# hila-chefer/Transformer-Explainability

Hardware: NVIDIA H100
Metric: explanations_per_sec (higher is better)
Workload: dtype f32

## Files before the change

transformer_explainability_b200/csrc/te_tc_wgmma.cu:

```cuda
#include <cuda.h>
#include <cuda_bf16.h>
#include <cuda_fp16.h>
#include <cuda_runtime.h>
#include <string.h>
#include <algorithm>
#include <string>
#include <type_traits>
#include <utility>

#include "te_gemm_tc.h"
#include "te_wgmma.cuh"

namespace {

constexpr int BM = 128, NTHREADS = 256;

__device__ __forceinline__ uint32_t smem_u32(const void* p) { return (uint32_t)__cvta_generic_to_shared(p); }
__device__ __forceinline__ void fence_proxy_async() { asm volatile("fence.proxy.async.shared::cta;" ::: "memory"); }
__device__ __forceinline__ void wg_fence() { asm volatile("wgmma.fence.sync.aligned;" ::: "memory"); }
__device__ __forceinline__ void wg_commit() { asm volatile("wgmma.commit_group.sync.aligned;" ::: "memory"); }
__device__ __forceinline__ void wg_wait0() { asm volatile("wgmma.wait_group.sync.aligned 0;" ::: "memory"); }
__device__ __forceinline__ void wg_wait1() { asm volatile("wgmma.wait_group.sync.aligned 1;" ::: "memory"); }

__device__ __forceinline__ void mbar_init(uint32_t bar, uint32_t count) {
    asm volatile("mbarrier.init.shared::cta.b64 [%0], %1;" ::"r"(bar), "r"(count) : "memory");
}
__device__ __forceinline__ void mbar_expect_tx(uint32_t bar, uint32_t bytes) {
    asm volatile("mbarrier.arrive.expect_tx.shared::cta.b64 _, [%0], %1;" ::"r"(bar), "r"(bytes) : "memory");
}
__device__ __forceinline__ void mbar_arrive(uint32_t bar) { asm volatile("mbarrier.arrive.shared::cta.b64 _, [%0];" ::"r"(bar) : "memory"); }
__device__ __forceinline__ void mbar_wait(uint32_t bar, uint32_t parity) {
    uint32_t done;
    do {
        asm volatile("{\n.reg .pred p;\nmbarrier.try_wait.parity.shared::cta.b64 p, [%1], %2;\nselp.u32 %0, 1, 0, p;\n}\n"
                     : "=r"(done) : "r"(bar), "r"(parity) : "memory");
    } while (!done);
}
__device__ __forceinline__ void tma_load(uint32_t dst, const CUtensorMap* map, int k, int row, uint32_t bar) {
    asm volatile("cp.async.bulk.tensor.2d.shared::cluster.global.tile.mbarrier::complete_tx::bytes [%0], [%1, {%2, %3}], [%4];"
                 ::"r"(dst), "l"((uint64_t)map), "r"(k), "r"(row), "r"(bar) : "memory");
}
__device__ __forceinline__ void tma_load3(uint32_t dst, const CUtensorMap* map, int x, int y, int z, uint32_t bar) {
    asm volatile("cp.async.bulk.tensor.3d.shared::cluster.global.tile.mbarrier::complete_tx::bytes [%0], [%1, {%2, %3, %4}], [%5];"
                 ::"r"(dst), "l"((uint64_t)map), "r"(x), "r"(y), "r"(z), "r"(bar) : "memory");
}
__device__ __forceinline__ void bar_named(int id, int threads) { asm volatile("bar.sync %0, %1;" ::"r"(id), "r"(threads) : "memory"); }
template <int N>
__device__ __forceinline__ void setmaxnreg_dec() { asm volatile("setmaxnreg.dec.sync.aligned.u32 %0;" ::"n"(N)); }
template <int N>
__device__ __forceinline__ void setmaxnreg_inc() { asm volatile("setmaxnreg.inc.sync.aligned.u32 %0;" ::"n"(N)); }

__device__ __forceinline__ float to_tf32(float x) {
    uint32_t u;
    asm("cvt.rna.tf32.f32 %0, %1;" : "=r"(u) : "f"(x));
    return __uint_as_float(u);
}
__device__ __forceinline__ float4 tf32x4(float4 v) { return make_float4(to_tf32(v.x), to_tf32(v.y), to_tf32(v.z), to_tf32(v.w)); }
__device__ __forceinline__ float4 absx4(float4 v) { return make_float4(fabsf(v.x), fabsf(v.y), fabsf(v.z), fabsf(v.w)); }
__device__ __forceinline__ float4 posx4(float4 v) { return make_float4(fmaxf(v.x, 0.f), fmaxf(v.y, 0.f), fmaxf(v.z, 0.f), fmaxf(v.w, 0.f)); }
__device__ __forceinline__ float4 negx4(float4 v) { return make_float4(fminf(v.x, 0.f), fminf(v.y, 0.f), fminf(v.z, 0.f), fminf(v.w, 0.f)); }
__device__ __forceinline__ float4 subx4(float4 a, float4 b) { return make_float4(a.x - b.x, a.y - b.y, a.z - b.z, a.w - b.w); }

__device__ __forceinline__ float ex2_approx(float x) {
    float y;
    asm("ex2.approx.ftz.f32 %0, %1;" : "=f"(y) : "f"(x));
    return y;
}

__device__ __forceinline__ uint32_t swz(int r, int c) { return (uint32_t)r * 128u + ((uint32_t)(c ^ (r & 7)) << 4); }

__device__ __forceinline__ uint64_t sdesc(uint32_t saddr) {
    uint64_t d = (uint64_t)((saddr & 0x3FFFFu) >> 4);
    d |= (uint64_t)1 << 16;
    d |= (uint64_t)(1024 >> 4) << 32;
    d |= (uint64_t)1 << 62;
    return d;
}

constexpr int TILE128 = 128 * 128;

template <int ACC, int A, int B>
struct Pr {
    static constexpr int acc = ACC, a = A, b = B;
};
template <class... T>
struct Prods {
    static constexpr int N = sizeof...(T), NACC = 1 + std::max({T::acc...});
    static constexpr int NTA = 1 + std::max({T::a...}), NTB = 1 + std::max({T::b...});
    __host__ __device__ static constexpr bool first(int i) {
        constexpr int acc[] = {T::acc...};
        for (int j = 0; j < i; ++j)
            if (acc[j] == acc[i]) return false;
        return true;
    }
};
using One = Prods<Pr<0, 0, 0>>;
using Split3 = Prods<Pr<0, 1, 0>, Pr<0, 0, 1>, Pr<0, 0, 0>>;

// ... 57 lines not shown
    const float4 h = tf32x4(v);
    st4(hi, r, c, h);
    st4(lo, r, c, tf32x4(subx4(v, h)));
}

template <class F>
__device__ __forceinline__ void map_rows(uint8_t* tile, int r0, int n, int t, int nt, F f) {
    float4* a = reinterpret_cast<float4*>(tile + r0 * 128);
    for (int i = t; i < n * 8; i += nt) a[i] = f(a[i]);
}
__device__ __forceinline__ void split_rows(uint8_t* hi, uint8_t* lo, int r0, int n, int t, int nt) {
    float4* h = reinterpret_cast<float4*>(hi + r0 * 128);
    float4* l = reinterpret_cast<float4*>(lo + r0 * 128);
    for (int i = t; i < n * 8; i += nt) {
        const float4 v = h[i], vh = tf32x4(v);
        h[i] = vh;
        l[i] = tf32x4(subx4(v, vh));
    }
}
template <class F>
__device__ __forceinline__ void transpose_rows(const uint8_t* land, int r0, int n, int t, int nt, F f) {
    for (int i = t; i < n * 8; i += nt) {
        const int r = r0 + i % n, c = i / n, m = r & 31;
        const uint8_t* box = land + (r >> 5) * 4096 + (m & 3) * 4;
        float e[4];
#pragma unroll
        for (int u = 0; u < 4; ++u) {
            const int k = 4 * c + u;
            e[u] = *reinterpret_cast<const float*>(box + k * 128 + (((m >> 2) ^ (k & 7)) << 4));
        }
        f(r, c, make_float4(e[0], e[1], e[2], e[3]));
    }
}
template <bool SP>
__device__ __forceinline__ auto put_tf32(uint8_t* hi, uint8_t* lo) {
    return [=](int r, int c, float4 v) {
        if (SP) st4(hi, r, c, tf32x4(v));
        else st_split(hi, lo, r, c, v);
    };
}
template <bool SP>
__device__ __forceinline__ void fix_tf32(uint8_t* hi, uint8_t* lo, int r0, int n, int t, int nt) {
    if (SP) map_rows(hi, r0, n, t, nt, [](float4 v) { return tf32x4(v); });
    else split_rows(hi, lo, r0, n, t, nt);
}

__device__ __forceinline__ int frag_row(int tid, int j) { return 64 * (tid >> 7) + 16 * ((tid >> 5) & 3) + ((tid & 31) >> 2) + 8 * ((j >> 1) & 1); }
__device__ __forceinline__ int frag_col(int tid, int j) { return 8 * (j >> 2) + 2 * (tid & 3) + (j & 1); }

constexpr int TMA_MAPS = 5;
struct TmaArgs {
    CUtensorMap map[TMA_MAPS];
    int mtiles, ntiles, nz;
};
enum { FIX_NONE = 0, FIX_A = 1, FIX_AB = 2 };
constexpr int NTHREADS_TMA = 384, SMEM_MAX = 227 * 1024;
__host__ __device__ constexpr int tma_stages(int bytes, int epi) {
    return (SMEM_MAX - 1024 - 256 - epi) / bytes < 8 ? (SMEM_MAX - 1024 - 256 - epi) / bytes : 8;
}

template <class P>
__host__ __device__ constexpr int epi_bytes() { return P::EPI_MAPS * BM * P::BN * 4; }
__device__ __forceinline__ float2 epi_f2(const uint8_t* t, int r, int c) {
    return *reinterpret_cast<const float2*>(t + (c >> 5) * (BM * 128) + swz(r, (c & 31) >> 2) + (c & 3) * 4);
}

template <class P, int NA, int NR, int NT, int NTR>
__device__ __forceinline__ void fold(const P& p, float (&acc)[NA][NR], float (&tot)[NT][NTR], int m0, int ch, int z, int tid) {
    const float s0 = p.chunk_scale(m0 + frag_row(tid, 0), ch, z), s1 = p.chunk_scale(m0 + frag_row(tid, 2), ch, z);
#pragma unroll
    for (int a = 0; a < NA; ++a)
#pragma unroll
        for (int j = 0; j < NR; ++j) tot[a][j] = fmaf(acc[a][j], ((j >> 1) & 1) ? s1 : s0, tot[a][j]);
}
template <int NA, int NR>
__device__ __forceinline__ void zero(float (&v)[NA][NR]) {
#pragma unroll
    for (int a = 0; a < NA; ++a)
#pragma unroll
        for (int j = 0; j < NR; ++j) v[a][j] = 0.f;
}

template <class P>
__device__ __forceinline__ void reg_tile(const P& p, uint8_t* smem, int col_fast) {
    constexpr int NR = P::BN / 2;
    constexpr int NA = P::PRODS::NACC;
    constexpr int STAGE = P::L::BYTES;
    constexpr int NT = P::CHUNK ? NA : 1, NTR = P::CHUNK ? NR : 1;
    const int tid = threadIdx.x, wg = tid >> 7;
    const int m0 = (col_fast ? blockIdx.y : blockIdx.x) * BM, n0 = (col_fast ? blockIdx.x : blockIdx.y) * P::BN;
    const int z = blockIdx.z;
    float acc[NA][NR];
    float tot[NT][NTR];
    zero(acc);
    zero(tot);

    const int kb = p.kblocks();
    p.load(smem, 0, m0, n0, z, tid);
    fence_proxy_async();
    __syncthreads();
    for (int it = 0; it < kb; ++it) {
        const bool fresh = P::CHUNK ? (it % P::CHUNK == 0) : (it == 0);
        wg_fence();
        issue<P>(smem_u32(smem + (it & 1) * STAGE), wg, acc, fresh ? 0u : 1u);
        wg_commit();
        if (it + 1 < kb) p.load(smem + ((it + 1) & 1) * STAGE, it + 1, m0, n0, z, tid);
        wg_wait0();
        if constexpr (P::CHUNK > 0)
            if ((it + 1) % P::CHUNK == 0 || it + 1 == kb) fold(p, acc, tot, m0, it / P::CHUNK, z, tid);
        fence_proxy_async();
        __syncthreads();
    }
    if constexpr (P::CHUNK > 0) p.epilogue(tot, m0, n0, z, tid, nullptr);
    else p.epilogue(acc, m0, n0, z, tid, nullptr);
}

template <class P>
__device__ __forceinline__ void tma_tiles(const P& p, const TmaArgs& ta, uint8_t* smem) {
    using L = typename P::L;
    constexpr int NR = P::BN / 2;
    constexpr int NA = P::PRODS::NACC;
    constexpr int STAGE = L::BYTES, EPI = epi_bytes<P>(), S = tma_stages(STAGE, EPI);
    constexpr int NT = P::CHUNK ? NA : 1, NTR = P::CHUNK ? NR : 1;
    static_assert(S >= 2, "a TMA problem needs two stages");
    __shared__ __align__(8) uint64_t bars[2 * S + 2];
    const int tid = threadIdx.x, wg = tid >> 7;
    const uint32_t full0 = smem_u32(bars), empty0 = full0 + 8u * S, st0 = smem_u32(smem);
    const uint32_t efull = full0 + 16u * S, eempty = efull + 8u, ebuf = st0 + (uint32_t)S * STAGE;
    if (tid == 0) {
        for (int s = 0; s < S; ++s) {
            mbar_init(full0 + 8u * s, 1);
            mbar_init(empty0 + 8u * s, 8);
        }
        mbar_init(efull, 1);
        mbar_init(eempty, 8);
        asm volatile("fence.mbarrier_init.release.cluster;" ::: "memory");
    }
    __syncthreads();
    const int kb = p.kblocks(), per_z = ta.mtiles * ta.ntiles, ntiles = ta.nz * per_z;
    int stage = 0;
    uint32_t phase = 0;
    auto decode = [&](int t, int& m0, int& n0, int& z) {
        z = t / per_z;
        const int r = t - z * per_z;
        m0 = (r / ta.ntiles) * BM;
        n0 = (r % ta.ntiles) * P::BN;
    };

    if (wg == 2) {
        setmaxnreg_dec<40>();
        if (tid != 2 * 128) return;
        uint32_t ephase = 0;
        for (int t = blockIdx.x; t < ntiles; t += gridDim.x) {
            int m0, n0, z;
            decode(t, m0, n0, z);
            for (int it = 0; it < kb; ++it) {
                mbar_wait(empty0 + 8u * stage, phase ^ 1u);
                p.produce(ta, st0 + (uint32_t)stage * STAGE, full0 + 8u * stage, it, m0, n0, z);
                if (++stage == S) { stage = 0; phase ^= 1u; }
                if constexpr (EPI > 0) {
                    if (it == min(S, kb) - 1) {
                        mbar_wait(eempty, ephase ^ 1u);
                        mbar_expect_tx(efull, EPI);
#pragma unroll
                        for (int i = 0; i < P::EPI_MAPS; ++i)
#pragma unroll
                            for (int b = 0; b < P::BN / 32; ++b)
                                tma_load(ebuf + (uint32_t)(i * BM * P::BN * 4 + b * BM * 128), &ta.map[P::NMAPS + i], n0 + 32 * b,
                                         m0, efull);
                        ephase ^= 1u;
                    }
                }
            }
        }
        return;
    }

    setmaxnreg_inc<232>();
    float acc[NA][NR];
    float tot[NT][NTR];
    auto release = [&](int s) {
        if ((tid & 31) == 0) mbar_arrive(empty0 + 8u * s);
    };
    auto consume = [&](uint32_t sd) {
        mbar_wait(full0 + 8u * stage, phase);
        if constexpr (P::FIX != FIX_NONE) {
            p.fix(smem + (uint32_t)stage * STAGE, wg, tid);
            fence_proxy_async();
            if constexpr (P::FIX == FIX_A) bar_named(1 + wg, 128);
            else bar_named(3, 256);
        }
        wg_fence();
        issue<P>(st0 + (uint32_t)stage * STAGE, wg, acc, sd);
        wg_commit();
    };
    auto next = [&] {
        if (++stage == S) { stage = 0; phase ^= 1u; }
    };
    constexpr int CH = P::CHUNK;
    uint32_t ephase = 0;
    for (int t = blockIdx.x; t < ntiles; t += gridDim.x) {
        int m0, n0, z;
        decode(t, m0, n0, z);
        zero(acc);
        zero(tot);
        for (int k0 = 0; k0 < kb; k0 += CH ? CH : kb) {
            const int k1 = CH ? min(k0 + CH, kb) : kb;
            consume(0u);
            for (int it = k0 + 1; it < k1; ++it) {
                const int prev = stage;
                next();
                consume(1u);
                wg_wait1();
                release(prev);
            }
            wg_wait0();
            release(stage);
            next();
            if constexpr (CH > 0) fold(p, acc, tot, m0, k0 / CH, z, tid);
        }
        if constexpr (EPI > 0) mbar_wait(efull, ephase);
        if constexpr (P::CHUNK > 0) p.epilogue(tot, m0, n0, z, tid, smem + (uint32_t)S * STAGE);
        else p.epilogue(acc, m0, n0, z, tid, smem + (uint32_t)S * STAGE);
        if constexpr (EPI > 0) {
            __syncwarp();
            if ((tid & 31) == 0) mbar_arrive(eempty);
            ephase ^= 1u;
        }
    }
}

template <class P>
__global__ void __launch_bounds__(P::TMA ? NTHREADS_TMA : NTHREADS, 1)
    wg_kernel(const P p, const __grid_constant__ TmaArgs ta, int col_fast) {
    extern __shared__ uint8_t smem_raw[];
    uint8_t* smem = smem_raw + ((1024u - (smem_u32(smem_raw) & 1023u)) & 1023u);
    if constexpr (P::TMA) tma_tiles(p, ta, smem);
    else reg_tile(p, smem, col_fast);
}

struct NoScale {
    __device__ __forceinline__ float chunk_scale(int, int, int) const { return 1.f; }
};

struct TmaTile {
    const void* base;
    long long rows, cols, ld;
    int box_rows;
    long long count = 0, cstride = 0;
};
template <class P>
__device__ __forceinline__ void produce_tiles(const TmaArgs& ta, uint32_t st, uint32_t bar, int it, int m0, int n0) {
    using L = typename P::L;
    constexpr int KE = P::FMT == OP_TF32 ? 32 : 64;
    mbar_expect_tx(bar, L::BYTES);
#pragma unroll
    for (int i = 0; i < L::NTA; ++i) tma_load(st + L::a(i), &ta.map[i], it * KE, m0, bar);
#pragma unroll
    for (int j = 0; j < L::NTB; ++j) tma_load(st + L::b(j), &ta.map[L::NTA + j], it * KE, n0, bar);
}
#define TE_PRODUCE_TILES(P)                                                                                      \
    static constexpr int NMAPS = L::NTA + L::NTB;                                                                \
    __device__ void produce(const TmaArgs& ta, uint32_t st, uint32_t bar, int it, int m0, int n0, int) const { \
        produce_tiles<P>(ta, st, bar, it, m0, n0);                                                               \
    }

enum { ZO_F32 = 0, ZO_BF16 = 1, ZO_F16S = 2 };
template <bool SINGLE, bool BF, int OUT>
struct ZsProb : NoScale {
    static constexpr int BN = 128, CHUNK = 0, FMT = BF ? OP_BF16 : OP_TF32;
    using PRODS = std::conditional_t<SINGLE, One, Prods<Pr<0, 0, 0>, Pr<0, 1, 1>>>;
    using L = Stage<PRODS, BN>;
    static constexpr bool COL_FAST = true;
    static constexpr bool TMA = SINGLE;
    static constexpr int FIX = SINGLE && !BF ? FIX_A : FIX_NONE;
    static constexpr int EPI_MAPS = SINGLE ? 2 : 0;
    int M, N, K;
    const float* x; long long ldx;
    const void* xabs;
    const void* wa; const void* wb;
    const float* r; long long ldr; const float* y; long long ldy; const float* bias;
    void* out; long long ldo; float* hs;
    float sscale, zsign;

    __device__ int kblocks() const { return K / (BF ? 64 : 32); }
    __device__ void fix(uint8_t* st, int wg, int tid) const {
        map_rows(st + L::a(0), 64 * wg, 64, tid & 127, 128, [](float4 v) { return tf32x4(absx4(v)); });
    }
    TE_PRODUCE_TILES(ZsProb)
    TmaTile tile(int i) const {
        if (i == 0) return BF ? TmaTile{xabs, M, K, K, BM} : TmaTile{x, M, K, ldx, BM};
        if (i == 1) return TmaTile{wa, N, K, K, BN};
        return i == 2 ? TmaTile{r, M, N, ldr, BM} : TmaTile{y, M, N, ldy, BM};
    }
    __device__ void load(uint8_t* st, int kb, int m0, int n0, int, int tid) const {
        for_k32(BM, x, ldx, m0, M, kb * 32, K, tid, [&](int rr, int c, float4 v) {
            st4(st + L::a(0), rr, c, tf32x4(posx4(v)));
            st4(st + L::a(1), rr, c, tf32x4(negx4(v)));
        });
        for_k32(BN, (const float*)wa, K, n0, N, kb * 32, K, tid, [&](int rr, int c, float4 v) { st4(st + L::b(0), rr, c, v); });
        for_k32(BN, (const float*)wb, K, n0, N, kb * 32, K, tid, [&](int rr, int c, float4 v) { st4(st + L::b(1), rr, c, v); });
    }
    __device__ void epilogue(float (&acc)[1][BN / 2], int m0, int n0, int, int tid, const uint8_t* eb) const {
        float sv[BN / 2];
        float rmax[2] = {0.f, 0.f};
#pragma unroll
        for (int j = 0; j < BN / 2; j += 2) {
            const int row = m0 + frag_row(tid, j), col = n0 + frag_col(tid, j);
            float2 rr = make_float2(0.f, 0.f), z = make_float2(acc[0][j], acc[0][j + 1]);
            if (row < M) {
                rr = SINGLE ? epi_f2(eb, frag_row(tid, j), frag_col(tid, j))
                            : *reinterpret_cast<const float2*>(r + (long long)row * ldr + col);
                if (SINGLE) {
                    const float2 yy = epi_f2(eb + BM * BN * 4, frag_row(tid, j), frag_col(tid, j));
                    const float2 bb = bias ? *reinterpret_cast<const float2*>(bias + col) : make_float2(0.f, 0.f);
                    z.x = 0.5f * ((yy.x - bb.x) + zsign * z.x);
                    z.y = 0.5f * ((yy.y - bb.y) + zsign * z.y);
                    z = zsign > 0.f ? make_float2(fmaxf(z.x, 0.f), fmaxf(z.y, 0.f)) : make_float2(fminf(z.x, 0.f), fminf(z.y, 0.f));
                }
            }
            sv[j] = sscale * te_sd(rr.x, z.x);
            sv[j + 1] = sscale * te_sd(rr.y, z.y);
            if (OUT == ZO_F16S) rmax[(j >> 1) & 1] = fmaxf(rmax[(j >> 1) & 1], fmaxf(fabsf(sv[j]), fabsf(sv[j + 1])));
        }
#pragma unroll
        for (int j = 0; j < BN / 2; j += 2) {
            const int row = m0 + frag_row(tid, j), col = n0 + frag_col(tid, j);
            if (row >= M) continue;
            if (OUT == ZO_F32) {
                *reinterpret_cast<float2*>((float*)out + (long long)row * ldo + col) = make_float2(to_tf32(sv[j]), to_tf32(sv[j + 1]));
            } else if (OUT == ZO_BF16) {
                *reinterpret_cast<__nv_bfloat162*>((__nv_bfloat16*)out + (long long)row * ldo + col) = __floats2bfloat162_rn(sv[j], sv[j + 1]);
            }
        }
        if (OUT == ZO_F16S) {
            float sc[2];
#pragma unroll
            for (int h = 0; h < 2; ++h) {
                float m = rmax[h];
                m = fmaxf(m, __shfl_xor_sync(0xffffffffu, m, 1));
                m = fmaxf(m, __shfl_xor_sync(0xffffffffu, m, 2));
                float si;
                te_f16_block_scale(m, sc[h], si);
                const int row = m0 + frag_row(tid, 2 * h);
                if ((tid & 3) == 0 && row < M) hs[(long long)row * (N / 128) + n0 / 128] = si;
            }
#pragma unroll
            for (int j = 0; j < BN / 2; j += 2) {
                const int row = m0 + frag_row(tid, j), col = n0 + frag_col(tid, j);
                const float s = sc[(j >> 1) & 1];
                if (row < M) *reinterpret_cast<__half2*>((__half*)out + (long long)row * N + col) = __floats2half2_rn(sv[j] * s, sv[j + 1] * s);
            }
        }
    }
};

template <int KIND>
struct ZrProb {
    static constexpr int BN = (KIND == 2) ? 64 : 128, CHUNK = (KIND == 2) ? 2 : 0;
    static constexpr int FMT = KIND == 0 ? OP_TF32 : KIND == 1 ? OP_BF16 : OP_F16;
    using PRODS = Prods<Pr<0, 0, 0>, Pr<1, 0, 1>>;
    using L = Stage<PRODS, BN>;
    static constexpr bool TMA = true;
    static constexpr int FIX = FIX_NONE, EPI_MAPS = KIND == 0 ? 0 : 1;
    int M, N, K;
    const void* s; const void* wp; const void* wn;
    const float* rs; int rs_ld; const float* cp; const float* cn;
    const float* x; long long ldx; float* out; long long ldo;
    int accum;

    __device__ int kblocks() const { return K / (KIND ? 64 : 32); }
    TE_PRODUCE_TILES(ZrProb)
    __device__ float chunk_scale(int row, int ch, int) const { return (KIND == 2 && row < M) ? rs[(long long)row * rs_ld + ch] : 1.f; }
    TmaTile tile(int i) const {
        if (i == 0) return TmaTile{s, M, K, K, BM};
        return i < 3 ? TmaTile{i == 1 ? wp : wn, N, K, K, BN} : TmaTile{x, M, N, ldx, BM};
    }
    __device__ void epilogue(float (&acc)[2][BN / 2], int m0, int n0, int, int tid, const uint8_t* eb) const {
#pragma unroll
        for (int j = 0; j < BN / 2; j += 2) {
            const int row = m0 + frag_row(tid, j), col = n0 + frag_col(tid, j);
            if (row >= M) continue;
            const float2 xv = EPI_MAPS ? epi_f2(eb, frag_row(tid, j), frag_col(tid, j))
                                       : *reinterpret_cast<const float2*>(x + (long long)row * ldx + col);
            float2 ap = make_float2(acc[0][j], acc[0][j + 1]), an = make_float2(acc[1][j], acc[1][j + 1]);
            if (KIND == 2) {
                ap.x *= cp[col]; ap.y *= cp[col + 1];
                an.x *= cn[col]; an.y *= cn[col + 1];
            }
            float2 v = make_float2(fmaxf(xv.x, 0.f) * ap.x + fminf(xv.x, 0.f) * an.x, fmaxf(xv.y, 0.f) * ap.y + fminf(xv.y, 0.f) * an.y);
            if (accum) {
                const float2 prev = *reinterpret_cast<const float2*>(out + (long long)row * ldo + col);
                v = make_float2(prev.x + v.x, prev.y + v.y);
            }
            acc[0][j] = v.x;
            acc[0][j + 1] = v.y;
        }
#pragma unroll
        for (int j = 0; j < BN / 2; j += 2) {
            const int row = m0 + frag_row(tid, j), col = n0 + frag_col(tid, j);
            if (row < M) *reinterpret_cast<float2*>(out + (long long)row * ldo + col) = make_float2(acc[0][j], acc[0][j + 1]);
        }
    }
};

template <bool NEG>
struct LrpSProb : NoScale {
    static constexpr int BN = 128, CHUNK = 0, FMT = OP_TF32;
    using PRODS = One;
    using L = Stage<PRODS, BN>;
    static constexpr bool COL_FAST = true, TMA = false;
    int M, N, K;
    const float* x; long long ldx; const float* w;
    const float* r; long long ldr; float* out;
    float sscale;
    __device__ int kblocks() const { return K / 32; }
    __device__ void load(uint8_t* st, int kb, int m0, int n0, int, int tid) const {
        for_k32(BM, x, ldx, m0, M, kb * 32, K, tid, [&](int rr, int c, float4 v) { st4(st + L::a(0), rr, c, tf32x4(NEG ? negx4(v) : posx4(v))); });
        for_k32(BN, w, K, n0, N, kb * 32, K, tid, [&](int rr, int c, float4 v) { st4(st + L::b(0), rr, c, v); });
    }
    __device__ void epilogue(float (&acc)[1][BN / 2], int m0, int n0, int, int tid, const uint8_t*) const {
#pragma unroll
        for (int j = 0; j < BN / 2; j += 2) {
            const int row = m0 + frag_row(tid, j), col = n0 + frag_col(tid, j);
            if (row >= M) continue;
            const float2 rr = *reinterpret_cast<const float2*>(r + (long long)row * ldr + col);
            *reinterpret_cast<float2*>(out + (long long)row * N + col) =
                make_float2(to_tf32(sscale * te_sd(rr.x, acc[0][j])), to_tf32(sscale * te_sd(rr.y, acc[0][j + 1])));
        }
    }
};
template <bool NEG>
struct LrpRProb : NoScale {
    static constexpr int BN = 128, CHUNK = 0, FMT = OP_TF32;
    using PRODS = One;
    using L = Stage<PRODS, BN>;
    static constexpr bool TMA = true;
    static constexpr int FIX = FIX_NONE, EPI_MAPS = 1;
    int M, N, K;
    const float* s; const float* wt;
    const float* x; long long ldx; float* out; long long ldo;
    int accum;
    __device__ int kblocks() const { return K / 32; }
    TE_PRODUCE_TILES(LrpRProb)
    TmaTile tile(int i) const {
        return i == 0 ? TmaTile{s, M, K, K, BM} : i == 1 ? TmaTile{wt, N, K, K, BN} : TmaTile{x, M, N, ldx, BM};
    }
    __device__ void epilogue(float (&acc)[1][BN / 2], int m0, int n0, int, int tid, const uint8_t* eb) const {
#pragma unroll
        for (int j = 0; j < BN / 2; j += 2) {
            const int row = m0 + frag_row(tid, j), col = n0 + frag_col(tid, j);
            if (row >= M) continue;
            const float2 xv = epi_f2(eb, frag_row(tid, j), frag_col(tid, j));
            const float2* o = reinterpret_cast<const float2*>(out + (long long)row * ldo + col);
            float2 v;
            if (NEG) {
                const float2 prev = *o;
                v = make_float2(prev.x + fminf(xv.x, 0.f) * acc[0][j], prev.y + fminf(xv.y, 0.f) * acc[0][j + 1]);
            } else if (accum) {
                const float2 prev = *o;
                v = make_float2(prev.x + fmaxf(xv.x, 0.f) * acc[0][j], prev.y + fmaxf(xv.y, 0.f) * acc[0][j + 1]);
            } else {
                v = make_float2(fmaxf(xv.x, 0.f) * acc[0][j], fmaxf(xv.y, 0.f) * acc[0][j + 1]);
            }
            acc[0][j] = v.x;
            acc[0][j + 1] = v.y;
        }
#pragma unroll
        for (int j = 0; j < BN / 2; j += 2) {
            const int row = m0 + frag_row(tid, j), col = n0 + frag_col(tid, j);
            if (row < M) *reinterpret_cast<float2*>(out + (long long)row * ldo + col) = make_float2(acc[0][j], acc[0][j + 1]);
        }
    }
};

struct LinOut {
    int M, N;
    const float* bias; const float* E; long long lde;
    float* C; long long ldc; float* C2; long long ldc2;
};
template <int EPI, bool FAST_GRAD, class EF>
__device__ __forceinline__ float2 lin_value(const LinOut& o, int col, float v0, float v1, EF e) {
    float2 b = make_float2(0.f, 0.f);
    if ((EPI == TE_TC_EPI_BIAS || EPI == TE_TC_EPI_BIAS_GELU || EPI == TE_TC_EPI_BIAS_ADD) && o.bias)
        b = *reinterpret_cast<const float2*>(o.bias + col);
    if (EPI == TE_TC_EPI_GELU_BWD) {
        const float2 ev = e();
        if (FAST_GRAD) return make_float2(v0 * te_gelu_grad_fast(ev.x), v1 * te_gelu_grad_fast(ev.y));
        return make_float2(v0 * te_gelu_grad(ev.x), v1 * te_gelu_grad(ev.y));
    }
    return make_float2(v0 + b.x, v1 + b.y);
}
template <int EPI, class EF>
__device__ __forceinline__ void lin_store(const LinOut& o, int row, int col, float2 y, EF e) {
    *reinterpret_cast<float2*>(o.C + (long long)row * o.ldc + col) = y;
    float2 y2 = make_float2(0.f, 0.f);
    if (EPI == TE_TC_EPI_BIAS_GELU) y2 = make_float2(te_gelu(y.x), te_gelu(y.y));
    if (EPI == TE_TC_EPI_BIAS_ADD) {
        const float2 ev = e();
        y2 = make_float2(ev.x + y.x, ev.y + y.y);
    }
    if (EPI == TE_TC_EPI_BIAS_GELU || EPI == TE_TC_EPI_BIAS_ADD) *reinterpret_cast<float2*>(o.C2 + (long long)row * o.ldc2 + col) = y2;
}

enum { LIN_3XTF32 = 0, LIN_TF32 = 1, LIN_F16X3 = 2, LIN_F16 = 3 };
struct LinArgs {
    int K, rs_ld;
    const void* a; const void* a_lo; long long lda;
    const void* b; const void* b_lo;
    const float* rs; const float* cs;
    LinOut o;
};
static_assert(sizeof(LinArgs) <= 128, "LinArgs: keep the kernel parameter within 128 bytes");
template <int EPI, int FORM>
struct LinProb : LinArgs {
    static constexpr bool F16 = FORM == LIN_F16X3 || FORM == LIN_F16, SPLIT = FORM == LIN_3XTF32 || FORM == LIN_F16X3;
    static constexpr int BN = FORM == LIN_TF32 && EPI == TE_TC_EPI_STORE ? 256 : 128;
    static constexpr int CHUNK = F16 ? 2 : SPLIT ? 4 : 0, FMT = F16 ? OP_F16 : OP_TF32;
    using PRODS = std::conditional_t<SPLIT, Split3, One>;
    using L = Stage<PRODS, BN>;
    static constexpr bool COL_FAST = true;
    static constexpr bool TMA = FORM != LIN_3XTF32;
    static constexpr int FIX = FORM == LIN_TF32 ? FIX_A : FIX_NONE;
    static constexpr int EPI_MAPS = TMA && EPI == TE_TC_EPI_GELU_BWD ? 1 : 0;
    __device__ int kblocks() const { return K / (F16 ? 64 : 32); }
    __device__ float chunk_scale(int row, int ch, int) const {
        if constexpr (F16) return row < o.M ? rs[(long long)row * rs_ld + ch] : 1.f;
        else return 1.f;
    }
    __device__ void fix(uint8_t* st, int wg, int tid) const {
        map_rows(st + L::a(0), 64 * wg, 64, tid & 127, 128, [](float4 v) { return tf32x4(v); });
    }
    TE_PRODUCE_TILES(LinProb)
    TmaTile tile(int i) const {
        if (i < L::NTA) return TmaTile{i == 0 ? a : a_lo, o.M, K, F16 ? K : lda, BM};
        if (i < NMAPS) return TmaTile{i == L::NTA ? b : b_lo, o.N, K, K, BN};
        return TmaTile{o.E, o.M, o.N, o.lde, BM};
    }
    __device__ void load(uint8_t* st, int kb, int m0, int n0, int, int tid) const {
        for_k32(BM, (const float*)a, lda, m0, o.M, kb * 32, K, tid, [&](int r, int c, float4 v) { st_split(st + L::a(0), st + L::a(1), r, c, v); });
        for_k32(BN, (const float*)b, K, n0, o.N, kb * 32, K, tid, [&](int r, int c, float4 v) { st4(st + L::b(0), r, c, v); });
        for_k32(BN, (const float*)b_lo, K, n0, o.N, kb * 32, K, tid, [&](int r, int c, float4 v) { st4(st + L::b(1), r, c, v); });
    }
    __device__ void epilogue(float (&acc)[1][BN / 2], int m0, int n0, int, int tid, const uint8_t* eb) const {
        auto inside = [&](int row, int col) { return row < o.M && (BN == 128 || col < o.N); };
        constexpr bool E_FIRST = EPI == TE_TC_EPI_BIAS_ADD && EPI_MAPS == 0;
        float2 ef[E_FIRST ? BN / 4 : 1];
#pragma unroll
        for (int j = 0; j < BN / 2; j += 2) {
            const int row = m0 + frag_row(tid, j), col = n0 + frag_col(tid, j);
            if (!inside(row, col)) continue;
            if constexpr (E_FIRST) ef[j / 2] = efrag(eb, tid, j, row, col);
            auto e = [&] { return efrag(eb, tid, j, row, col); };
            float2 y;
            if constexpr (F16)
                y = lin_value<EPI, false>(o, col, acc[0][j] * cs[col], acc[0][j + 1] * cs[col + 1], e);
            else y = lin_value<EPI, FORM == LIN_TF32>(o, col, acc[0][j], acc[0][j + 1], e);
            acc[0][j] = y.x;
            acc[0][j + 1] = y.y;
        }
#pragma unroll
        for (int j = 0; j < BN / 2; j += 2) {
            const int row = m0 + frag_row(tid, j), col = n0 + frag_col(tid, j);
            if (inside(row, col))
                lin_store<EPI>(o, row, col, make_float2(acc[0][j], acc[0][j + 1]), [&] {
                    if constexpr (E_FIRST) return ef[j / 2];
                    else return efrag(eb, tid, j, row, col);
                });
        }
    }
    __device__ float2 efrag(const uint8_t* eb, int tid, int j, int row, int col) const {
        if constexpr (EPI_MAPS > 0) return epi_f2(eb, frag_row(tid, j), frag_col(tid, j));
        else return *reinterpret_cast<const float2*>(o.E + (long long)row * o.lde + col);
    }
};

enum { AT_STORE = 0, AT_MUL = 1, AT_SD = 2, AT_SOFTMAX = 3, AT_RESID = 4 };
template <int EPI, bool SP, int BN_>
struct NnProb : NoScale {
    static constexpr int BN = BN_, CHUNK = 0, FMT = OP_TF32;
    using PRODS = std::conditional_t<SP, One, Split3>;
    using L = Stage<PRODS, BN>;
    static constexpr bool TMA = true;
    static constexpr int FIX = FIX_AB, EPI_MAPS = 0;
    int N, H, dh, ld_out, batch;
    const float* a; long long lda; const float* b; long long ldb;
    const float* E; float* out; float alpha;
    __device__ int kblocks() const { return dh / 32; }
    static constexpr int NMAPS = 2;
    TmaTile tile(int i) const {
        return i == 0 ? TmaTile{a, (long long)batch * N, H * dh, lda, BM} : TmaTile{b, (long long)batch * N, H * dh, ldb, BN};
    }
    __device__ void produce(const TmaArgs& ta, uint32_t st, uint32_t bar, int kb, int m0, int n0, int bh) const {
        const int s = bh / H, k = (bh % H) * dh + kb * 32;
        mbar_expect_tx(bar, TILE128 + BN * 128);
        tma_load(st + L::a(0), &ta.map[0], k, s * N + m0, bar);
        tma_load(st + L::b(0), &ta.map[1], k, s * N + n0, bar);
    }
    __device__ void fix(uint8_t* st, int wg, int tid) const {
        fix_tf32<SP>(st + L::a(0), st + L::a(1), 64 * wg, 64, tid & 127, 128);
        fix_tf32<SP>(st + L::b(0), st + L::b(1), 0, BN, tid, 256);
    }
    __device__ void epilogue(float (&acc)[1][BN / 2], int m0, int n0, int bh, int tid, const uint8_t*) const {
        const int ncols = (N + 3) & ~3;
        if constexpr (EPI == AT_SOFTMAX) {
            float mx[2] = {-INFINITY, -INFINITY};
#pragma unroll
            for (int j = 0; j < BN / 2; ++j)
                if (n0 + frag_col(tid, j) < N) mx[(j >> 1) & 1] = fmaxf(mx[(j >> 1) & 1], alpha * acc[0][j]);
            float sum[2] = {0.f, 0.f}, m2[2];
#pragma unroll
            for (int h = 0; h < 2; ++h) {
                mx[h] = fmaxf(mx[h], __shfl_xor_sync(0xffffffffu, mx[h], 1));
                mx[h] = fmaxf(mx[h], __shfl_xor_sync(0xffffffffu, mx[h], 2));
                m2[h] = -mx[h] * 1.4426950408889634f;
            }
            const float a2 = alpha * 1.4426950408889634f;
#pragma unroll
            for (int j = 0; j < BN / 2; ++j) {
                const float e = (n0 + frag_col(tid, j) < N) ? ex2_approx(fmaf(a2, acc[0][j], m2[(j >> 1) & 1])) : 0.f;
                acc[0][j] = e;
                sum[(j >> 1) & 1] += e;
            }
#pragma unroll
            for (int h = 0; h < 2; ++h) {
                sum[h] += __shfl_xor_sync(0xffffffffu, sum[h], 1);
                sum[h] += __shfl_xor_sync(0xffffffffu, sum[h], 2);
                sum[h] = 1.0f / sum[h];
            }
#pragma unroll
            for (int j = 0; j < BN / 2; j += 2) {
                const int r = m0 + frag_row(tid, j), col = n0 + frag_col(tid, j);
                if (r >= N || col >= ncols) continue;
                const float inv = sum[(j >> 1) & 1];
                *reinterpret_cast<float2*>(out + ((long long)bh * N + r) * ld_out + col) = make_float2(acc[0][j] * inv, acc[0][j + 1] * inv);
            }
        } else {
        float2 ef[BN / 4];
#pragma unroll
        for (int j = 0; j < BN / 2; j += 2) {
            const int r = m0 + frag_row(tid, j), col = n0 + frag_col(tid, j);
            ef[j / 2] = (EPI != AT_STORE && r < N && col < ncols)
                            ? *reinterpret_cast<const float2*>(E + ((long long)bh * N + r) * ld_out + col) : make_float2(0.f, 0.f);
        }
#pragma unroll
        for (int j = 0; j < BN / 2; j += 2) {
            const int r = m0 + frag_row(tid, j), col = n0 + frag_col(tid, j);
            if (r >= N || col >= ncols) continue;
            const long long off = ((long long)bh * N + r) * ld_out + col;
            const float2 e = ef[j / 2];
            float v[2] = {alpha * acc[0][j], alpha * acc[0][j + 1]};
            const float ee[2] = {e.x, e.y};
#pragma unroll
            for (int u = 0; u < 2; ++u) {
                if (EPI == AT_MUL) v[u] *= ee[u];
                else if (EPI == AT_SD) v[u] = te_sd_fast(ee[u], v[u]);
                if (col + u >= N) v[u] = 0.f;
            }
            *reinterpret_cast<float2*>(out + off) = make_float2(v[0], v[1]);
        }
        }
    }
};

template <int AMN, int EPI, bool SP, int BN_>
struct NkProb : NoScale {
    static constexpr int BN = BN_, CHUNK = SP ? 0 : 4, FMT = OP_TF32;
    using PRODS = std::conditional_t<SP, One, Split3>;
    static constexpr int LAND_A = AMN ? BM * 128 : 0, LAND_X = BN * 128;
    using L = Stage<PRODS, BN, LAND_A + LAND_X>;
    static constexpr bool TMA = true;
    static constexpr int FIX = FIX_AB, EPI_MAPS = 0;
    int N, H, NP, ld_out, n_out, n_pad, a_shared, batch;
    const float* map; const float* X; long long ldx;
    const float* rowscale; const float* E; float* out; float alpha;
    __device__ int kblocks() const { return (N + 31) / 32; }
    static constexpr int NMAPS = 2;
    TmaTile tile(int i) const {
        if (i == 0) return TmaTile{map, N, N, NP, AMN ? 32 : BM, (long long)batch * (a_shared ? 1 : H), (long long)N * NP};
        return TmaTile{X, N, n_pad, ldx, 32, batch, (long long)N * ldx};
    }
    __device__ void produce(const TmaArgs& ta, uint32_t st, uint32_t bar, int kb, int m0, int, int bh) const {
        const int s = bh / H, h = bh % H, za = a_shared ? s : bh;
        mbar_expect_tx(bar, (AMN ? LAND_A : TILE128) + LAND_X);
        if (AMN == 0) tma_load3(st + L::a(0), &ta.map[0], kb * 32, m0, za, bar);
#pragma unroll
        for (int j = 0; j < LAND_A / 4096; ++j) tma_load3(st + L::land() + j * 4096, &ta.map[0], m0 + 32 * j, kb * 32, za, bar);
#pragma unroll
        for (int j = 0; j < LAND_X / 4096; ++j)
            tma_load3(st + L::land() + LAND_A + j * 4096, &ta.map[1], h * BN + 32 * j, kb * 32, s, bar);
    }
    __device__ void fix(uint8_t* st, int wg, int tid) const {
        if (AMN) transpose_rows(st + L::land(), 64 * wg, 64, tid & 127, 128, put_tf32<SP>(st + L::a(0), st + L::a(1)));
        else fix_tf32<SP>(st + L::a(0), st + L::a(1), 64 * wg, 64, tid & 127, 128);
        transpose_rows(st + L::land() + LAND_A, 0, BN, tid, 256, put_tf32<SP>(st + L::b(0), st + L::b(1)));
    }
    __device__ void epilogue(float (&acc)[1][BN / 2], int m0, int, int bh, int tid, const uint8_t*) const {
        const int s = bh / H, h = bh % H;
        float2 ef[BN / 4];
#pragma unroll
        for (int j = 0; j < BN / 2; j += 2) {
            const int m = m0 + frag_row(tid, j), gcol = h * BN + frag_col(tid, j);
            ef[j / 2] = (EPI != AT_STORE && m < N && gcol < n_pad)
                            ? *reinterpret_cast<const float2*>(E + ((long long)s * N + m) * ld_out + gcol) : make_float2(0.f, 0.f);
        }
#pragma unroll
        for (int j = 0; j < BN / 2; j += 2) {
            const int m = m0 + frag_row(tid, j), gcol = h * BN + frag_col(tid, j);
            if (m >= N || gcol >= n_pad) continue;
            const long long off = ((long long)s * N + m) * ld_out + gcol;
            float v[2] = {alpha * acc[0][j], alpha * acc[0][j + 1]};
            const float2 e = ef[j / 2];
            if (EPI == AT_MUL) {
                v[0] *= e.x; v[1] *= e.y;
            } else if (EPI == AT_RESID) {
                const float rsc = rowscale ? rowscale[(long long)s * N + m] : 1.f;
                v[0] += rsc * e.x; v[1] += rsc * e.y;
            }
            if (gcol >= n_out) v[0] = 0.f;
            if (gcol + 1 >= n_out) v[1] = 0.f;
            *reinterpret_cast<float2*>(out + off) = make_float2(v[0], v[1]);
        }
    }
};

inline bool a16(const void* p) { return ((uintptr_t)p & 15u) == 0; }

int sm_count() {
    static int sms[64];
    int dev = 0;
    cudaGetDevice(&dev);
    int& n = sms[dev & 63];
    if (n == 0 && cudaDeviceGetAttribute(&n, cudaDevAttrMultiProcessorCount, dev) != cudaSuccess) n = 1;
    return n;
}

using EncodeTiled = CUresult (*)(CUtensorMap*, CUtensorMapDataType, cuuint32_t, void*, const cuuint64_t*, const cuuint64_t*,
                                 const cuuint32_t*, const cuuint32_t*, CUtensorMapInterleave, CUtensorMapSwizzle,
                                 CUtensorMapL2promotion, CUtensorMapFloatOOBfill);
EncodeTiled encode_tiled() {
    static const EncodeTiled fn = [] {
        void* f = nullptr;
        cudaDriverEntryPointQueryResult q;
        if (cudaGetDriverEntryPoint("cuTensorMapEncodeTiled", &f, cudaEnableDefault, &q) != cudaSuccess ||
            q != cudaDriverEntryPointSuccess)
            return (EncodeTiled) nullptr;
        return (EncodeTiled)f;
    }();
    return fn;
}
bool encode_tile(CUtensorMap* map, const TmaTile& t, int esize) {
    const EncodeTiled fn = encode_tiled();
    const int rank = t.count > 0 ? 3 : 2;
    if (!fn || ((uintptr_t)t.base & 15u) || (t.ld * esize) % 16 != 0 || (t.cstride * esize) % 16 != 0 || t.rows < 1 || t.cols < 1)
        return false;
    const cuuint64_t dims[3] = {(cuuint64_t)t.cols, (cuuint64_t)t.rows, (cuuint64_t)t.count};
    const cuuint64_t strides[2] = {(cuuint64_t)(t.ld * esize), (cuuint64_t)(t.cstride * esize)};
    const cuuint32_t box[3] = {(cuuint32_t)(128 / esize), (cuuint32_t)t.box_rows, 1}, estr[3] = {1, 1, 1};
    return fn(map, esize == 4 ? CU_TENSOR_MAP_DATA_TYPE_FLOAT32 : CU_TENSOR_MAP_DATA_TYPE_UINT16, rank, const_cast<void*>(t.base),
              dims, strides, box, estr, CU_TENSOR_MAP_INTERLEAVE_NONE, CU_TENSOR_MAP_SWIZZLE_128B,
              CU_TENSOR_MAP_L2_PROMOTION_L2_256B, CU_TENSOR_MAP_FLOAT_OOB_FILL_NONE) == CUDA_SUCCESS;
}

template <class P>
int launch(const P& p, dim3 grid, cudaStream_t st) {
    TmaArgs ta;
    memset(&ta, 0, sizeof(ta));
    int col_fast = 0, threads = NTHREADS, smem = 2 * P::L::BYTES + 1024;
    if constexpr (P::TMA) {
        constexpr int ESIZE = P::FMT == OP_TF32 ? 4 : 2;
        static_assert(P::NMAPS + P::EPI_MAPS <= TMA_MAPS, "TmaArgs holds TMA_MAPS tensor maps");
        for (int i = 0; i < P::NMAPS + P::EPI_MAPS; ++i)
            if (!encode_tile(&ta.map[i], p.tile(i), i < P::NMAPS ? ESIZE : 4)) {
                te_set_last_error("te_tc: cannot encode a TMA tensor map (16-byte-aligned base and strides required)");
                return TE_ERR_ARG;
            }
        const long long tiles = (long long)grid.x * grid.y * grid.z;
        if (tiles > INT32_MAX) { te_set_last_error("te_tc: grid too large for one launch"); return TE_ERR_ARG; }
        ta.mtiles = (int)grid.x;
        ta.ntiles = (int)grid.y;
        ta.nz = (int)grid.z;
        grid = dim3((unsigned)std::min<long long>(tiles, sm_count()));
        threads = NTHREADS_TMA;
        smem = tma_stages(P::L::BYTES, epi_bytes<P>()) * P::L::BYTES + epi_bytes<P>() + 1024;
    } else {
        col_fast = P::COL_FAST && grid.x <= 65535;
        if (col_fast) grid = dim3(grid.y, grid.x, grid.z);
    }
    static unsigned long long done = 0;
    int dev = 0;
    if (cudaGetDevice(&dev) != cudaSuccess) { te_set_last_error("te_tc: cudaGetDevice failed"); return TE_ERR_CUDA; }
    if (!(done & (1ull << (dev & 63)))) {
        if (cudaFuncSetAttribute(wg_kernel<P>, cudaFuncAttributeMaxDynamicSharedMemorySize, smem) != cudaSuccess) {
            te_set_last_error("te_tc: cannot raise dynamic shared memory");
            return TE_ERR_CUDA;
        }
        done |= 1ull << (dev & 63);
    }
    if (grid.y > 65535 || grid.z > 65535) { te_set_last_error("te_tc: grid too large for one launch"); return TE_ERR_ARG; }
    wg_kernel<P><<<grid, threads, smem, st>>>(p, ta, col_fast);
    TE_CUDA_CHECK_LAUNCH();
    return TE_OK;
}
inline unsigned mtiles(long long M) { return (unsigned)((M + BM - 1) / BM); }

__global__ void prepare_weights_kernel(const float* __restrict__ w, float* __restrict__ d, int out_f, int in_f) {
    const TeDerived<float> dv(d, in_f, out_f);
    __shared__ float tile[32][33];
    const int bx = blockIdx.x * 32, by = blockIdx.y * 32;
    for (int i = threadIdx.y; i < 32; i += blockDim.y) {
        const int o = by + i, c = bx + threadIdx.x;
        float v = 0.f;
        if (o < out_f && c < in_f) {
            const long long idx = (long long)o * in_f + c;
            v = w[idx];
            dv.wp[idx] = to_tf32(fmaxf(v, 0.f));
            dv.wn[idx] = to_tf32(fminf(v, 0.f));
            const float hi = to_tf32(v);
            dv.wh[idx] = hi;
            dv.wl[idx] = to_tf32(v - hi);
            dv.wabs[idx] = to_tf32(fabsf(v));
            dv.bf_wabs[idx] = __float2bfloat16_rn(fabsf(v));
        }
        tile[i][threadIdx.x] = v;
    }
    __syncthreads();
    for (int i = threadIdx.y; i < 32; i += blockDim.y) {
        const int c = bx + i, o = by + threadIdx.x;
        if (o < out_f && c < in_f) {
            const float v = tile[threadIdx.x][i];
            const long long idx = (long long)c * out_f + o;
            dv.wpt[idx] = to_tf32(fmaxf(v, 0.f));
            dv.wnt[idx] = to_tf32(fminf(v, 0.f));
            dv.bf_wpt[idx] = __float2bfloat16_rn(fmaxf(v, 0.f));
            dv.bf_wnt[idx] = __float2bfloat16_rn(fminf(v, 0.f));
            const float hi = to_tf32(v);
            dv.wth[idx] = hi;
// ... 434 lines not shown
```

Before: 923.1.

## Stage GEMM epilogue outputs in shared memory and write them with TMA stores

For several wgmma GEMM variants (attention score store/SD, GELU-backward linear, and the bf16 single-output product), the consumer warpgroups now write results into a swizzled shared-memory tile. The producer thread then issues asynchronous TMA bulk tensor stores for that tile, overlapped with the next tile's mainloop, instead of each thread issuing scattered float2 global stores. This adds an output tensor map, a shared-memory epilogue buffer where one did not exist before (which can reduce the number of pipeline stages), and a wait on store reads before the buffer is reused.

```diff
diff --git a/transformer_explainability_b200/csrc/te_tc_wgmma.cu b/transformer_explainability_b200/csrc/te_tc_wgmma.cu
--- a/transformer_explainability_b200/csrc/te_tc_wgmma.cu
+++ b/transformer_explainability_b200/csrc/te_tc_wgmma.cu
@@ -44,6 +44,13 @@
     asm volatile("cp.async.bulk.tensor.3d.shared::cluster.global.tile.mbarrier::complete_tx::bytes [%0], [%1, {%2, %3, %4}], [%5];"
                  ::"r"(dst), "l"((uint64_t)map), "r"(x), "r"(y), "r"(z), "r"(bar) : "memory");
 }
+__device__ __forceinline__ void tma_store3(const CUtensorMap* map, uint32_t src, int x, int y, int z) {
+    asm volatile("cp.async.bulk.tensor.3d.global.shared::cta.bulk_group [%0, {%1, %2, %3}], [%4];"
+                 ::"l"((uint64_t)map), "r"(x), "r"(y), "r"(z), "r"(src) : "memory");
+}
+__device__ __forceinline__ void bulk_commit() { asm volatile("cp.async.bulk.commit_group;" ::: "memory"); }
+__device__ __forceinline__ void bulk_wait_read() { asm volatile("cp.async.bulk.wait_group.read 0;" ::: "memory"); }
+__device__ __forceinline__ void bulk_wait_all() { asm volatile("cp.async.bulk.wait_group 0;" ::: "memory"); }
 __device__ __forceinline__ void bar_named(int id, int threads) { asm volatile("bar.sync %0, %1;" ::"r"(id), "r"(threads) : "memory"); }
 template <int N>
 __device__ __forceinline__ void setmaxnreg_dec() { asm volatile("setmaxnreg.dec.sync.aligned.u32 %0;" ::"n"(N)); }
@@ -207,6 +214,7 @@
 struct TmaArgs {
     CUtensorMap map[TMA_MAPS];
     int mtiles, ntiles, nz;
+    int out_cols;
 };
 enum { FIX_NONE = 0, FIX_A = 1, FIX_AB = 2 };
 constexpr int NTHREADS_TMA = 384, SMEM_MAX = 227 * 1024;
@@ -216,9 +224,11 @@
 
 template <class P>
 __host__ __device__ constexpr int epi_bytes() { return P::EPI_MAPS * BM * P::BN * 4; }
-__device__ __forceinline__ float2 epi_f2(const uint8_t* t, int r, int c) {
-    return *reinterpret_cast<const float2*>(t + (c >> 5) * (BM * 128) + swz(r, (c & 31) >> 2) + (c & 3) * 4);
-}
+template <class P>
+__host__ __device__ constexpr int buf_bytes() { return (P::EPI_MAPS > 0 || !P::OUT_SMEM ? P::EPI_MAPS : 1) * BM * P::BN * 4; }
+__device__ __forceinline__ uint32_t epi_off(int r, int c) { return (c >> 5) * (BM * 128) + swz(r, (c & 31) >> 2) + (c & 3) * 4; }
+__device__ __forceinline__ float2 epi_f2(const uint8_t* t, int r, int c) { return *reinterpret_cast<const float2*>(t + epi_off(r, c)); }
+__device__ __forceinline__ void epi_st2(uint8_t* t, int r, int c, float2 v) { *reinterpret_cast<float2*>(t + epi_off(r, c)) = v; }
 
 template <class P, int NA, int NR, int NT, int NTR>
 __device__ __forceinline__ void fold(const P& p, float (&acc)[NA][NR], float (&tot)[NT][NTR], int m0, int ch, int z, int tid) {
@@ -275,7 +285,7 @@
     using L = typename P::L;
     constexpr int NR = P::BN / 2;
     constexpr int NA = P::PRODS::NACC;
-    constexpr int STAGE = L::BYTES, EPI = epi_bytes<P>(), S = tma_stages(STAGE, EPI);
+    constexpr int STAGE = L::BYTES, EPI = buf_bytes<P>(), S = tma_stages(STAGE, EPI);
     constexpr int NT = P::CHUNK ? NA : 1, NTR = P::CHUNK ? NR : 1;
     static_assert(S >= 2, "a TMA problem needs two stages");
     __shared__ __align__(8) uint64_t bars[2 * S + 2];
@@ -306,6 +316,15 @@
         setmaxnreg_dec<40>();
         if (tid != 2 * 128) return;
         uint32_t ephase = 0;
+        int om0 = -1, on0 = 0, oz = 0;
+        auto store_out = [&] {
+#pragma unroll
+            for (int b = 0; b < P::BN / 32; ++b)
+                if (on0 + 32 * b < ta.out_cols)
+                    tma_store3(&ta.map[P::NMAPS + P::EPI_MAPS], ebuf + (uint32_t)(b * BM * 128), on0 + 32 * b, om0, oz);
+            bulk_commit();
+            bulk_wait_read();
+        };
         for (int t = blockIdx.x; t < ntiles; t += gridDim.x) {
             int m0, n0, z;
             decode(t, m0, n0, z);
@@ -316,7 +335,14 @@
                 if constexpr (EPI > 0) {
                     if (it == min(S, kb) - 1) {
                         mbar_wait(eempty, ephase ^ 1u);
-                        mbar_expect_tx(efull, EPI);
+                        if constexpr (P::OUT_SMEM) {
+                            if (om0 >= 0) store_out();
+                            om0 = m0;
+                            on0 = n0;
+                            oz = z;
+                        }
+                        if constexpr (P::EPI_MAPS == 0) mbar_arrive(efull);
+                        else mbar_expect_tx(efull, EPI);
 #pragma unroll
                         for (int i = 0; i < P::EPI_MAPS; ++i)
 #pragma unroll
@@ -326,6 +352,13 @@
                         ephase ^= 1u;
                     }
                 }
+            }
+        }
+        if constexpr (P::OUT_SMEM) {
+            if (om0 >= 0) {
+                mbar_wait(eempty, ephase ^ 1u);
+                store_out();
+                bulk_wait_all();
             }
         }
         return;
@@ -378,6 +411,7 @@
         if constexpr (P::CHUNK > 0) p.epilogue(tot, m0, n0, z, tid, smem + (uint32_t)S * STAGE);
         else p.epilogue(acc, m0, n0, z, tid, smem + (uint32_t)S * STAGE);
         if constexpr (EPI > 0) {
+            if constexpr (P::OUT_SMEM) fence_proxy_async();
             __syncwarp();
             if ((tid & 31) == 0) mbar_arrive(eempty);
             ephase ^= 1u;
@@ -430,6 +464,7 @@
     static constexpr bool TMA = SINGLE;
     static constexpr int FIX = SINGLE && !BF ? FIX_A : FIX_NONE;
     static constexpr int EPI_MAPS = SINGLE ? 2 : 0;
+    static constexpr bool OUT_SMEM = SINGLE && BF && OUT == ZO_F32;
     int M, N, K;
     const float* x; long long ldx;
     const void* xabs;
@@ -446,7 +481,7 @@
     TmaTile tile(int i) const {
         if (i == 0) return BF ? TmaTile{xabs, M, K, K, BM} : TmaTile{x, M, K, ldx, BM};
         if (i == 1) return TmaTile{wa, N, K, K, BN};
-        return i == 2 ? TmaTile{r, M, N, ldr, BM} : TmaTile{y, M, N, ldy, BM};
+        return i == 2 ? TmaTile{r, M, N, ldr, BM} : i == 3 ? TmaTile{y, M, N, ldy, BM} : TmaTile{out, M, N, ldo, BM, 1, M * ldo};
     }
     __device__ void load(uint8_t* st, int kb, int m0, int n0, int, int tid) const {
         for_k32(BM, x, ldx, m0, M, kb * 32, K, tid, [&](int rr, int c, float4 v) {
@@ -456,7 +491,7 @@
         for_k32(BN, (const float*)wa, K, n0, N, kb * 32, K, tid, [&](int rr, int c, float4 v) { st4(st + L::b(0), rr, c, v); });
         for_k32(BN, (const float*)wb, K, n0, N, kb * 32, K, tid, [&](int rr, int c, float4 v) { st4(st + L::b(1), rr, c, v); });
     }
-    __device__ void epilogue(float (&acc)[1][BN / 2], int m0, int n0, int, int tid, const uint8_t* eb) const {
+    __device__ void epilogue(float (&acc)[1][BN / 2], int m0, int n0, int, int tid, uint8_t* eb) const {
         float sv[BN / 2];
         float rmax[2] = {0.f, 0.f};
 #pragma unroll
@@ -481,6 +516,10 @@
 #pragma unroll
         for (int j = 0; j < BN / 2; j += 2) {
             const int row = m0 + frag_row(tid, j), col = n0 + frag_col(tid, j);
+            if (OUT_SMEM) {
+                epi_st2(eb, frag_row(tid, j), frag_col(tid, j), make_float2(to_tf32(sv[j]), to_tf32(sv[j + 1])));
+                continue;
+            }
             if (row >= M) continue;
             if (OUT == ZO_F32) {
                 *reinterpret_cast<float2*>((float*)out + (long long)row * ldo + col) = make_float2(to_tf32(sv[j]), to_tf32(sv[j + 1]));
@@ -518,6 +557,7 @@
     using L = Stage<PRODS, BN>;
     static constexpr bool TMA = true;
     static constexpr int FIX = FIX_NONE, EPI_MAPS = KIND == 0 ? 0 : 1;
+    static constexpr bool OUT_SMEM = false;
     int M, N, K;
     const void* s; const void* wp; const void* wn;
     const float* rs; int rs_ld; const float* cp; const float* cn;
@@ -592,6 +632,7 @@
     using L = Stage<PRODS, BN>;
     static constexpr bool TMA = true;
     static constexpr int FIX = FIX_NONE, EPI_MAPS = 1;
+    static constexpr bool OUT_SMEM = false;
     int M, N, K;
     const float* s; const float* wt;
     const float* x; long long ldx; float* out; long long ldo;
@@ -678,6 +719,7 @@
     static constexpr bool TMA = FORM != LIN_3XTF32;
     static constexpr int FIX = FORM == LIN_TF32 ? FIX_A : FIX_NONE;
     static constexpr int EPI_MAPS = TMA && EPI == TE_TC_EPI_GELU_BWD ? 1 : 0;
+    static constexpr bool OUT_SMEM = FORM == LIN_TF32 && EPI == TE_TC_EPI_GELU_BWD;
     __device__ int kblocks() const { return K / (F16 ? 64 : 32); }
     __device__ float chunk_scale(int row, int ch, int) const {
         if constexpr (F16) return row < o.M ? rs[(long long)row * rs_ld + ch] : 1.f;
@@ -690,14 +732,14 @@
     TmaTile tile(int i) const {
         if (i < L::NTA) return TmaTile{i == 0 ? a : a_lo, o.M, K, F16 ? K : lda, BM};
         if (i < NMAPS) return TmaTile{i == L::NTA ? b : b_lo, o.N, K, K, BN};
-        return TmaTile{o.E, o.M, o.N, o.lde, BM};
+        return i < NMAPS + EPI_MAPS ? TmaTile{o.E, o.M, o.N, o.lde, BM} : TmaTile{o.C, o.M, o.N, o.ldc, BM, 1, (long long)o.M * o.ldc};
     }
     __device__ void load(uint8_t* st, int kb, int m0, int n0, int, int tid) const {
         for_k32(BM, (const float*)a, lda, m0, o.M, kb * 32, K, tid, [&](int r, int c, float4 v) { st_split(st + L::a(0), st + L::a(1), r, c, v); });
         for_k32(BN, (const float*)b, K, n0, o.N, kb * 32, K, tid, [&](int r, int c, float4 v) { st4(st + L::b(0), r, c, v); });
         for_k32(BN, (const float*)b_lo, K, n0, o.N, kb * 32, K, tid, [&](int r, int c, float4 v) { st4(st + L::b(1), r, c, v); });
     }
-    __device__ void epilogue(float (&acc)[1][BN / 2], int m0, int n0, int, int tid, const uint8_t* eb) const {
+    __device__ void epilogue(float (&acc)[1][BN / 2], int m0, int n0, int, int tid, uint8_t* eb) const {
         auto inside = [&](int row, int col) { return row < o.M && (BN == 128 || col < o.N); };
         constexpr bool E_FIRST = EPI == TE_TC_EPI_BIAS_ADD && EPI_MAPS == 0;
         float2 ef[E_FIRST ? BN / 4 : 1];
@@ -717,7 +759,8 @@
 #pragma unroll
         for (int j = 0; j < BN / 2; j += 2) {
             const int row = m0 + frag_row(tid, j), col = n0 + frag_col(tid, j);
-            if (inside(row, col))
+            if constexpr (OUT_SMEM) epi_st2(eb, frag_row(tid, j), frag_col(tid, j), make_float2(acc[0][j], acc[0][j + 1]));
+            else if (inside(row, col))
                 lin_store<EPI>(o, row, col, make_float2(acc[0][j], acc[0][j + 1]), [&] {
                     if constexpr (E_FIRST) return ef[j / 2];
                     else return efrag(eb, tid, j, row, col);
@@ -738,13 +781,16 @@
     using L = Stage<PRODS, BN>;
     static constexpr bool TMA = true;
     static constexpr int FIX = FIX_AB, EPI_MAPS = 0;
+    static constexpr bool OUT_SMEM = EPI == AT_STORE || EPI == AT_SD;
     int N, H, dh, ld_out, batch;
     const float* a; long long lda; const float* b; long long ldb;
     const float* E; float* out; float alpha;
     __device__ int kblocks() const { return dh / 32; }
     static constexpr int NMAPS = 2;
     TmaTile tile(int i) const {
-        return i == 0 ? TmaTile{a, (long long)batch * N, H * dh, lda, BM} : TmaTile{b, (long long)batch * N, H * dh, ldb, BN};
+        if (i == 0) return TmaTile{a, (long long)batch * N, H * dh, lda, BM};
+        if (i == 1) return TmaTile{b, (long long)batch * N, H * dh, ldb, BN};
+        return TmaTile{out, N, (N + 3) & ~3, ld_out, BM, (long long)batch * H, (long long)N * ld_out};
     }
     __device__ void produce(const TmaArgs& ta, uint32_t st, uint32_t bar, int kb, int m0, int n0, int bh) const {
         const int s = bh / H, k = (bh % H) * dh + kb * 32;
@@ -756,7 +802,7 @@
         fix_tf32<SP>(st + L::a(0), st + L::a(1), 64 * wg, 64, tid & 127, 128);
         fix_tf32<SP>(st + L::b(0), st + L::b(1), 0, BN, tid, 256);
     }
-    __device__ void epilogue(float (&acc)[1][BN / 2], int m0, int n0, int bh, int tid, const uint8_t*) const {
+    __device__ void epilogue(float (&acc)[1][BN / 2], int m0, int n0, int bh, int tid, uint8_t* ob) const {
         const int ncols = (N + 3) & ~3;
         if constexpr (EPI == AT_SOFTMAX) {
             float mx[2] = {-INFINITY, -INFINITY};
@@ -801,8 +847,7 @@
 #pragma unroll
         for (int j = 0; j < BN / 2; j += 2) {
             const int r = m0 + frag_row(tid, j), col = n0 + frag_col(tid, j);
-            if (r >= N || col >= ncols) continue;
-            const long long off = ((long long)bh * N + r) * ld_out + col;
+            if (!OUT_SMEM && (r >= N || col >= ncols)) continue;
             const float2 e = ef[j / 2];
             float v[2] = {alpha * acc[0][j], alpha * acc[0][j + 1]};
             const float ee[2] = {e.x, e.y};
@@ -812,7 +857,8 @@
                 else if (EPI == AT_SD) v[u] = te_sd_fast(ee[u], v[u]);
                 if (col + u >= N) v[u] = 0.f;
             }
-            *reinterpret_cast<float2*>(out + off) = make_float2(v[0], v[1]);
+            if (OUT_SMEM) epi_st2(ob, frag_row(tid, j), frag_col(tid, j), make_float2(v[0], v[1]));
+            else *reinterpret_cast<float2*>(out + ((long long)bh * N + r) * ld_out + col) = make_float2(v[0], v[1]);
         }
         }
     }
@@ -826,6 +872,7 @@
     using L = Stage<PRODS, BN, LAND_A + LAND_X>;
     static constexpr bool TMA = true;
     static constexpr int FIX = FIX_AB, EPI_MAPS = 0;
+    static constexpr bool OUT_SMEM = false;
     int N, H, NP, ld_out, n_out, n_pad, a_shared, batch;
     const float* map; const float* X; long long ldx;
     const float* rowscale; const float* E; float* out; float alpha;
@@ -924,8 +971,10 @@
     int col_fast = 0, threads = NTHREADS, smem = 2 * P::L::BYTES + 1024;
     if constexpr (P::TMA) {
         constexpr int ESIZE = P::FMT == OP_TF32 ? 4 : 2;
-        static_assert(P::NMAPS + P::EPI_MAPS <= TMA_MAPS, "TmaArgs holds TMA_MAPS tensor maps");
-        for (int i = 0; i < P::NMAPS + P::EPI_MAPS; ++i)
+        constexpr int NM = P::NMAPS + P::EPI_MAPS + (P::OUT_SMEM ? 1 : 0);
+        static_assert(NM <= TMA_MAPS, "TmaArgs holds TMA_MAPS tensor maps");
+        if constexpr (P::OUT_SMEM) ta.out_cols = (int)p.tile(NM - 1).cols;
+        for (int i = 0; i < NM; ++i)
             if (!encode_tile(&ta.map[i], p.tile(i), i < P::NMAPS ? ESIZE : 4)) {
                 te_set_last_error("te_tc: cannot encode a TMA tensor map (16-byte-aligned base and strides required)");
                 return TE_ERR_ARG;
@@ -937,7 +986,7 @@
         ta.nz = (int)grid.z;
         grid = dim3((unsigned)std::min<long long>(tiles, sm_count()));
         threads = NTHREADS_TMA;
-        smem = tma_stages(P::L::BYTES, epi_bytes<P>()) * P::L::BYTES + epi_bytes<P>() + 1024;
+        smem = tma_stages(P::L::BYTES, buf_bytes<P>()) * P::L::BYTES + buf_bytes<P>() + 1024;
     } else {
         col_fast = P::COL_FAST && grid.x <= 65535;
         if (col_fast) grid = dim3(grid.y, grid.x, grid.z);
```

After: 940.5, median of 6. +1.9%, better.
